# naver/panst3r

Measured on AMD Instinct MI355X. Metric: frames/sec (whole node), N-view 512px panoptic inference, higher is better.
Workload: dtype f16

## Files before the change

include/panst3r_hip.h:

```cpp
#ifndef PANST3R_HIP_H
#define PANST3R_HIP_H
#include <stdint.h>
#ifdef __cplusplus
extern "C" {
#endif

#define PST_ABI_VERSION 20

#define PST_BF16 0
#define PST_F32  1
#define PST_F16  2
#define PST_X3H  4

int pst_abi_version(void);
const char* pst_last_error(void);

typedef struct pst_gemm_params {
  const void* A;  int64_t lda;
  const void* W;  int64_t ldw;
  void* C;        int64_t ldc;
  int32_t M, N, K;
  const float* bias;
  const float* gamma;
  const float* res;  int64_t ldr;
  int32_t res_mod;
  int32_t act;
  int32_t out_fp32;
  int32_t trans_out;
  int32_t grp_in, grp_out, grp_off;
  int32_t ps_p, ps_c, ps_h, ps_w;
  int32_t conv_c, conv_h, conv_w;
  const void* zeros;
  const int32_t* rope_pos; const float* rope_cs; int32_t rope_hd;
  int32_t rope_npos;
  int32_t res_bf16;
  int32_t kernel;
  int32_t batch;
  int64_t a_bs, w_bs, c_bs, bias_bs;
  int32_t dtype16;
  void* xcopy; int64_t ldxc;
  float* stats_out; int32_t stats_ld;
  const float* ln_stats; int32_t ln_groups; const float* ln_colsum; float ln_eps;
  int32_t x3_block;
} pst_gemm_params;

int pst_gemm(const pst_gemm_params* p, void* stream);
const char* pst_gemm_variant(const pst_gemm_params* p);
int pst_gemm_pair(const pst_gemm_params* a, const pst_gemm_params* b, void* stream);
const char* pst_gemm_pair_variant(const pst_gemm_params* a, const pst_gemm_params* b);
#define PST_TUNE_G256_PP 3
#define PST_TUNE_PAIR 4
#define PST_TUNE_DEEP_RING 8
#define PST_TUNE_PAIR_ATTN 7
#define PST_TUNE_ATTN_XCD 9
#define PST_TUNE_CUS 10
#define PST_TUNE_PAIR_DELAY 6
#define PST_TUNE_DEPHASE 11
#define PST_TUNE_PAIR_RES 5
int pst_tune(int knob, int value);

int pst_mask_head_supported(int Q, int P, int C);
int pst_mask_head(const void* E, int64_t lde, const void* F, int64_t f_view_stride, float* out, int64_t out_view_stride, int nviews, int Q, int P, int C,
                  int dtype16, void* stream);

typedef struct pst_attn_params {
  const void* Q;  int64_t q_bs, q_hs, q_rs;
  const void* K;  int64_t k_bs, k_hs, k_rs;
  const void* Vt; int64_t v_bs, v_hs, v_ds;
  void* O;        int64_t o_bs, o_hs, o_rs;
  const uint8_t* mask; int64_t m_bs, m_rs;
// ... 154 lines not shown
```

panst3r_amd/csrc/gemm.hip:

```cpp
#include "common.h"
#include "../../include/panst3r_hip.h"

namespace pst {

int launch_gemm256(const pst_gemm_params& p, hipStream_t s);
int launch_gemm256p(const pst_gemm_params& p, hipStream_t s, int cus);
int gemm256p_pair_split(const pst_gemm_params& a, const pst_gemm_params& b, int cus, double separate_us, double* pair_us);
double gemm256p_single_us(const pst_gemm_params& p, int cus);
int launch_gemm256p_pair(const pst_gemm_params& a, const pst_gemm_params& b, hipStream_t s, int cus, int g0);
bool gemm256_persistent_ok(const pst_gemm_params& p);
int gemm256_persistent_class(const pst_gemm_params& p);
int gemm_f32_validate(const pst_gemm_params& p);
int launch_gemm_f32(const pst_gemm_params& p, hipStream_t s);
int rowstream_class(const pst_gemm_params& p);
int launch_rowstream(const pst_gemm_params& p, hipStream_t s, int cus);

constexpr int BK = 64;
constexpr int GROUP_M = 8;

template <int F>
__device__ __forceinline__ int perm_row(int row) {
  const int sub = row / (16 * F), rho = row - sub * (16 * F);
  const int f = rho >> 4, g = (rho >> 2) & 3, r = rho & 3;
  return sub * (16 * F) + g * (4 * F) + 4 * f + r;
// ... 38 lines not shown
    }
    uint4 rq[F32 ? 1 : NIT];
    if (!F32 && resb) {
#pragma unroll
      for (int it = 0; it < NIT; ++it) rq[F32 ? 0 : it] = *(const uint4*)((const bf16_t*)p.res + (int64_t)orow[it] * p.ldr + n);
    }
    if (rope) {
      constexpr int GRP = NIT < 4 ? NIT : 4;
#pragma unroll
      for (int g0 = 0; g0 < NIT; g0 += GRP) {
        float4 cs[GRP][4];
#pragma unroll
        for (int u = 0; u < GRP; ++u) rope_table(p, m0 + r0 + (g0 + u) * rstep, n, cs[u]);
#pragma unroll
        for (int u = 0; u < GRP; ++u) {
          const int r = r0 + (g0 + u) * rstep;
          const uint4 own = *(const uint4*)(smem + r * pitch + ((c ^ (r & (nch - 1))) << 4));
          const uint4 partner = *(const uint4*)(smem + r * pitch + (((c ^ 2) ^ (r & (nch - 1))) << 4));
          *(uint4*)((char*)p.C + ((int64_t)orow[g0 + u] * p.ldc + n) * 2) = rope_rotate<F16>(own, partner, cs[u], n);
        }
      }
      return;
    }
#pragma unroll
    for (int it = 0; it < NIT; ++it) {
      const int r = r0 + it * rstep;
      uint4 val = *(const uint4*)(smem + r * pitch + ((c ^ (r & (nch - 1))) << 4));
      if (F32 && pre) {
        float4 f = *(float4*)&val;
        const float4 q = resv[it];
        f.x += q.x; f.y += q.y; f.z += q.z; f.w += q.w;
        val = *(uint4*)&f;
      }
      float ssum = 0.f, ssq = 0.f;
      if (!F32 && resb) {
        uint32_t* w32 = (uint32_t*)&val;
        const uint32_t* q32 = (const uint32_t*)&rq[F32 ? 0 : it];
#pragma unroll
        for (int q = 0; q < 4; ++q) {
          w32[q] = H16<F16>::pack(H16<F16>::lo(w32[q]) + H16<F16>::lo(q32[q]), H16<F16>::hi(w32[q]) + H16<F16>::hi(q32[q]));
          if (p.stats_out) { ln_acc(H16<F16>::lo(w32[q]), ssum, ssq); ln_acc(H16<F16>::hi(w32[q]), ssum, ssq); }
        }
      } else if (!F32 && p.stats_out) {
        const uint32_t* w32 = (const uint32_t*)&val;
#pragma unroll
        for (int q = 0; q < 4; ++q) { ln_acc(H16<F16>::lo(w32[q]), ssum, ssq); ln_acc(H16<F16>::hi(w32[q]), ssum, ssq); }
      }
      if (F32) store_c4(p, orow[it], n, *(const float4*)&val);
      else *(uint4*)((char*)p.C + ((int64_t)orow[it] * p.ldc + n) * 2) = val;
      if (F32) {
        const float4 f = *(const float4*)&val;
        if (p.xcopy) *(uint2*)((bf16_t*)p.xcopy + (int64_t)orow[it] * p.ldxc + n) = make_uint2(H16<F16>::pack(f.x, f.y), H16<F16>::pack(f.z, f.w));
        if (p.stats_out) { float ss, sq; ln_acc4(f, ss, sq); ln_fold_stats<16>(p, ss, sq, c, orow[it], n); }
      } else if (p.stats_out) {
        ln_fold_stats<8>(p, ssum, ssq, c, orow[it], n);
      }
    }
    return;
  }
#pragma unroll
  for (int it = 0; it < (F32 ? BM / 8 : BM / 16); ++it) {
    const int r = tid / nch + it * rstep;
    const int m = m0 + r;
    if (r >= BM || m >= p.M || n >= p.N) continue;
    uint4 val = *(const uint4*)(smem + r * pitch + ((c ^ (r & (nch - 1))) << 4));
    if (p.rope_hd == 64 && !F32) val = rope_chunk<F16>(p, val, *(const uint4*)(smem + r * pitch + (((c ^ 2) ^ (r & (nch - 1))) << 4)), m, n);
    int orow = m;
    int64_t off;
    int ps_v = 0, ps_y = 0, ps_x = 0;
    if (p.ps_p > 0) {
      const int hw = p.ps_h * p.ps_w;
      ps_v = m / hw;
      const int tt = m - ps_v * hw;
      ps_y = tt / p.ps_w;
      ps_x = tt - ps_y * p.ps_w;
      const int dy = n / seg, rem = n - dy * seg;
      off = ((int64_t)(ps_v * p.ps_p * p.ps_h + p.ps_p * ps_y + dy) * p.ps_w + ps_x) * seg + rem;
    } else {
// ... 108 lines not shown
    if (p.conv_c > 0) {
      const int hw = p.conv_h * p.conv_w;
      const int img = m / hw, r = m - img * hw;
      const int y = r / p.conv_w;
      a_yx[j] = (y << 16) | (r - y * p.conv_w);
      a_src[j] = Ap + (int64_t)img * hw * p.conv_c;
    } else {
      a_yx[j] = 0;
      a_src[j] = Ap + (int64_t)m * p.lda;
    }
  }
#pragma unroll
  for (int j = 0; j < FN; ++j) {
    const int c = j * 256 + tid, lrow = c >> 3, pos = c & 7;
    b_sw[j] = ((pos ^ ((lrow >> 1) & 7)) << 3);
    const int row = TRANS ? lrow : perm_row<FN>(lrow);
    b_src[j] = Wp + (int64_t)min(n0 + row, p.N - 1) * p.ldw;
  }

  auto stage = [&](int kt, int buf) {
    const int k0 = kt * BK;
    char* a_dst = As + buf * (BM * 128) + wave * 1024;
    char* b_dst = Bs + buf * (BN * 128) + wave * 1024;
    if (p.conv_c > 0) {
      const int tap = k0 / p.conv_c, c0 = k0 - tap * p.conv_c;
      const int dy = tap / 3 - 1, dx = tap - (tap / 3) * 3 - 1;
#pragma unroll
      for (int j = 0; j < FM; ++j) {
        const int yy = (a_yx[j] >> 16) + dy, xx = (a_yx[j] & 0xffff) + dx;
        const bool ok = (yy >= 0) & (yy < p.conv_h) & (xx >= 0) & (xx < p.conv_w);
        const bf16_t* s = ok ? a_src[j] + ((int64_t)yy * p.conv_w + xx) * p.conv_c + c0 + a_sw[j]
                             : (const bf16_t*)p.zeros + a_sw[j];
        glds16(s, a_dst + j * 4096);
      }
    } else {
#pragma unroll
      for (int j = 0; j < FM; ++j) glds16(a_src[j] + k0 + a_sw[j], a_dst + j * 4096);
    }
#pragma unroll
    for (int j = 0; j < FN; ++j) glds16(b_src[j] + k0 + b_sw[j], b_dst + j * 4096);
  };

  f32x4 acc[FM][FN];
#pragma unroll
  for (int i = 0; i < FM; ++i)
#pragma unroll
    for (int j = 0; j < FN; ++j) acc[i][j] = f32x4{0.f, 0.f, 0.f, 0.f};
// ... 182 lines not shown
  hipLaunchKernelGGL((gemm_pair_kernel<FM, FN, NST, F16>), dim3(tma * tna + tmb * tnb), dim3(256), lds, s, a, tma * tna, tma, tna, b, tmb * tnb, tmb, tnb);
  return check_launch("gemm_pair");
}

template <int FM, int FN, bool TRANS, int NST, bool F16>
static int launch_t(const pst_gemm_params& p, hipStream_t s) {
  constexpr int BM = 32 * FM, BN = 32 * FN;
  const int tiles_m = (p.M + BM - 1) / BM, tiles_n = (p.N + BN - 1) / BN;
  const int tiles = tiles_m * tiles_n;
  const size_t lds = NST * (BM + BN) * 128 + BM * sizeof(float2);
  if constexpr (NST > 4) {
    static unsigned long long attr_seen = 0;
    once_per_device(attr_seen, [] { (void)hipFuncSetAttribute((const void*)gemm_kernel<FM, FN, TRANS, NST, F16>, hipFuncAttributeMaxDynamicSharedMemorySize, NST * (BM + BN) * 128 + BM * (int)sizeof(float2)); });
  }
  hipLaunchKernelGGL((gemm_kernel<FM, FN, TRANS, NST, F16>), dim3(tiles, p.batch > 1 ? p.batch : 1), dim3(256), lds, s, p, tiles, tiles_m, tiles_n);
  return check_launch("gemm");
}

template <int FM, int FN, bool TRANS, int NST>
static int launch(const pst_gemm_params& p, hipStream_t s) {
  return p.dtype16 == DT_F16 ? launch_t<FM, FN, TRANS, NST, true>(p, s) : launch_t<FM, FN, TRANS, NST, false>(p, s);
}

}

static int gemm_validate(const pst_gemm_params* pp) {
  using namespace pst;
  if (!pp) { set_error("gemm: null params"); return PST_EINVAL; }
  const pst_gemm_params& p = *pp;
  if (p.dtype16 == DT_F32) {
    if (p.M <= 0 || p.N <= 0 || p.K <= 0 || !p.A || !p.W || !p.C) { set_error("gemm: bad shape / null operand"); return PST_EINVAL; }
    if (p.kernel != 0) { set_error("gemm (fp32 operands): kernel must be 0"); return PST_EINVAL; }
    return pst::gemm_f32_validate(p);
  }
  if (p.dtype16 != DT_BF16 && p.dtype16 != DT_F16) { set_error("gemm: dtype16 must be PST_BF16, PST_F16 or PST_F32"); return PST_EINVAL; }
  if (p.act < 0 || p.act > 2) {
    set_error("gemm: act %d not available with 16-bit operands (0 none, 1 GELU(erf), 2 ReLU; 3 = GELU(tanh) needs fp32 operands)", p.act); return PST_EINVAL;
  }
  if (p.kernel != 0 && p.kernel != 128 && p.kernel != 256) { set_error("gemm: kernel must be 0 (auto), 128 or 256"); return PST_EINVAL; }
  if (p.kernel == 256 && (p.conv_c > 0 || (p.trans_out && pst::gemm256_persistent_class(p) != 3))) {
    set_error("gemm: the 256x256 kernel has no conv mode, and trans_out only in its persistent class (16-bit, ldc %% 8 == 0, N %% 64 == 0)"); return PST_EINVAL;
  }
  if (p.M <= 0 || p.N <= 0 || p.K <= 0) { set_error("gemm: bad shape M=%d N=%d K=%d", p.M, p.N, p.K); return PST_EINVAL; }
  if (p.K % 64 || p.N % 4) { set_error("gemm: need K%%64==0 and N%%4==0 (K=%d N=%d)", p.K, p.N); return PST_EINVAL; }
  if (!p.A || !p.W || !p.C) { set_error("gemm: null operand"); return PST_EINVAL; }
  if ((((uintptr_t)p.A | (uintptr_t)p.W) & 15) || ((uintptr_t)p.C & (p.out_fp32 ? 15 : 7))) {
    set_error("gemm: A/W must be 16-byte aligned, C 8-byte (bf16) / 16-byte (fp32) aligned"); return PST_EINVAL;
  }
  if ((p.ldw % 8) || (p.conv_c == 0 && (p.lda % 8))) { set_error("gemm: lda/ldw must be multiples of 8"); return PST_EINVAL; }
  if (p.conv_c > 0 && (p.conv_c % 64 || p.K != 9 * p.conv_c || !p.zeros || p.M % (p.conv_h * p.conv_w))) {
    set_error("gemm: bad conv mode (conv_c=%d K=%d)", p.conv_c, p.K); return PST_EINVAL;
  }
  if (p.ps_p > 0 && ((p.ps_p * p.ps_c) % 4 || p.N != p.ps_p * p.ps_p * p.ps_c || p.M % (p.ps_h * p.ps_w) || p.res || p.grp_in)) {
    set_error("gemm: bad pixel-shuffle store (p=%d c=%d N=%d)", p.ps_p, p.ps_c, p.N); return PST_EINVAL;
  }
  if (p.trans_out && (p.out_fp32 || p.res || p.gamma || p.grp_in || p.ps_p || (p.ldc % 4))) {
    set_error("gemm: trans_out supports bf16 + bias/act only, ldc%%4==0"); return PST_EINVAL;
  }
  if (!p.trans_out && !p.ps_p && (p.ldc % 4)) { set_error("gemm: ldc must be a multiple of 4"); return PST_EINVAL; }
  if (p.rope_hd != 0 && (p.rope_hd != 64 || p.out_fp32 || p.trans_out || p.ps_p || p.N % 64 || !p.rope_pos || !p.rope_cs || p.res)) {
    set_error("gemm: fused RoPE needs head dim 64, bf16 plain output, N%%64==0, no residual"); return PST_EINVAL;
  }
  if (p.res && (p.ldr % (p.res_bf16 ? 8 : 4))) { set_error("gemm: ldr must be a multiple of 4 (fp32) / 8 (bf16)"); return PST_EINVAL; }
  if (p.res && p.res_bf16 && ((uintptr_t)p.res & 15)) { set_error("gemm: bf16 residual must be 16-byte aligned"); return PST_EINVAL; }
  if ((p.stats_out || p.xcopy) && (p.N % 64 || p.ps_p || p.trans_out || p.res_mod || p.batch > 1 || (p.stats_out && p.stats_ld < p.N / 64) ||
                                   (p.xcopy && (!p.out_fp32 || p.ldxc % 4 || ((uintptr_t)p.xcopy & 7))))) {
    set_error("gemm: LayerNorm-fold producer outputs need a plain row-major store with N%%64==0 (xcopy: fp32 C only)"); return PST_EINVAL;
  }
  if (p.ln_stats && (!p.ln_colsum || p.ln_groups <= 0 || p.conv_c || p.batch > 1 || !(p.ln_eps > 0.f))) {
    set_error("gemm: LayerNorm-fold consumer needs ln_colsum, ln_groups > 0, ln_eps > 0 (no conv / batch mode)"); return PST_EINVAL;
  }
  if (p.x3_block && (!p.out_fp32 || p.dtype16 != DT_F16 || p.x3_block < p.N || p.x3_block % 4 || p.ldc < 3 * (int64_t)p.x3_block || p.ldc % 4 || p.ps_p || p.trans_out || p.xcopy ||
                     p.stats_out || p.batch > 1 || ((uintptr_t)p.C & 7))) {
    set_error("gemm: the split store (x3_block) needs out_fp32, f16 operands, x3_block >= N, ldc >= 3 x3_block, a plain row-major store"); return PST_EINVAL;
  }
  if (p.batch > 1 && (p.gamma || p.res || p.conv_c || p.rope_hd || p.ps_p || p.grp_in || p.kernel == 256 || p.batch > 65535 ||
                      (p.a_bs | p.w_bs | p.c_bs) % 8 || p.bias_bs % 4)) {
    set_error("gemm: strided batch supports bias/act/trans_out only, strides multiples of 8 elements (batch=%d)", p.batch); return PST_EINVAL;
  }
  return PST_OK;
}

static int g_deep_ring = 4;
namespace pst { int gemm256_pp(int set); int gemm256p_dephase(int set); int gemm256p_pair_delay(int set); int attn_pair_enable(int set); int attn_xcd_order(int set); }

static int gemm_choice(const pst_gemm_params& p) {
  const long big_tiles = (long)((p.M + 127) / 128) * ((p.N + 127) / 128) * (p.batch > 1 ? p.batch : 1);
  const bool small = p.kernel == 0 && big_tiles < (p.K >= 2048 ? 176 : 256);
  const long tiles256 = (long)((p.M + 255) / 256) * ((p.N + 255) / 256);
  const bool fits32 = (int64_t)p.M * p.lda < (1ll << 31) && (int64_t)p.N * p.ldw < (1ll << 31);
  const bool one_round = tiles256 >= 176 && tiles256 <= 256;
  if (p.trans_out) {
    const bool p3 = pst::gemm256_persistent_class(p) == 3 && fits32 && p.batch <= 1 && (p.kernel == 256 || (p.kernel == 0 && (tiles256 >= 384 || one_round) && p.K >= 512));
    return p3 ? 2 : (small ? 0 : 1);
  }
  const bool shape256 = p.N % 256 == 0 && p.K >= 1024 && (p.N >= 2048 || p.K >= 2048) && tiles256 >= 3 * 256 - 64;
  const int pclass = pst::gemm256_persistent_class(p);
  const bool shape256p = (tiles256 >= 384 || one_round) && ((pclass == 1 && p.K >= 512) || (pclass == 2 && (p.K >= 2048 || (p.K >= 768 && tiles256 <= 512))));
  if (p.conv_c == 0 && fits32 && p.batch <= 1 && (p.kernel == 256 || (p.kernel == 0 && (shape256 || shape256p)))) return 2;
  return small ? 0 : 1;
}

extern "C" int pst_gemm(const pst_gemm_params* pp, void* stream) {
  using namespace pst;
  if (int rc = gemm_validate(pp)) return rc;
  const pst_gemm_params& p = *pp;
  hipStream_t s = (hipStream_t)stream;
  if (p.dtype16 == DT_F32) return launch_gemm_f32(p, s);
  if (rowstream_class(p)) return launch_rowstream(p, s, num_cus());
  const int c = gemm_choice(p);
  if (c == 2) return gemm256_persistent_ok(p) ? launch_gemm256p(p, s, num_cus()) : launch_gemm256(p, s);
  if (p.trans_out) return c == 0 ? launch<2, 2, true, 4>(p, s) : launch<4, 4, true, 2>(p, s);
  if (c == 0 && g_deep_ring > 4 && p.batch <= 1) {
    const long tiles = (long)((p.M + 63) / 64) * ((p.N + 63) / 64);
    if (tiles <= num_cus() && p.K >= 512) return g_deep_ring >= 8 ? launch<2, 2, false, 8>(p, s) : launch<2, 2, false, 6>(p, s);
  }
  return c == 0 ? launch<2, 2, false, 4>(p, s) : launch<4, 4, false, 2>(p, s);
}

static bool pair_fusable(const pst_gemm_params& a, const pst_gemm_params& b) {
  using namespace pst;
  if (a.dtype16 == DT_F32 || a.dtype16 != b.dtype16 || a.trans_out || !b.trans_out || a.batch > 1 || b.batch > 1 || a.kernel || b.kernel) return false;
  if (rowstream_class(a) || rowstream_class(b)) return false;
  return gemm_choice(a) == 0 && gemm_choice(b) == 0;
}

static int g_pair_res = 1;
static int g_pair = 1;
static int pair_split_256p(const pst_gemm_params& a, const pst_gemm_params& b) {
  using namespace pst;
  if (!g_pair || a.dtype16 == DT_F32 || a.dtype16 != b.dtype16 || a.batch > 1 || b.batch > 1 || a.kernel || b.kernel) return 0;
  if (rowstream_class(a) || rowstream_class(b)) return 0;
  const int cus = num_cus();
  double sep = 0.0;
  const pst_gemm_params* ps[2] = {&a, &b};
  for (const pst_gemm_params* p : ps) {
    const bool fits32 = (int64_t)p->M * p->lda < (1ll << 31) && (int64_t)p->N * p->ldw < (1ll << 31);
    if (gemm_choice(*p) == 2 && gemm256_persistent_ok(*p)) { sep += gemm256p_single_us(*p, cus); continue; }
    const long tiles256 = (long)((p->M + 255) / 256) * ((p->N + 255) / 256);
    if (!(g_pair_res && gemm256_persistent_class(*p) == 2 && fits32 && p->conv_c == 0 && p->K >= 1024 && tiles256 >= 128)) return 0;
    sep += 2.0 * p->M * p->N * p->K / 470e6;
  }
  return gemm256p_pair_split(a, b, cus, sep, nullptr);
}

extern "C" int pst_gemm_pair(const pst_gemm_params* pa, const pst_gemm_params* pb, void* stream) {
  using namespace pst;
  if (int rc = gemm_validate(pa)) return rc;
  if (int rc = gemm_validate(pb)) return rc;
  hipStream_t s = (hipStream_t)stream;
  if (const int g0 = pair_split_256p(*pa, *pb)) return launch_gemm256p_pair(*pa, *pb, s, num_cus(), g0);
  if (!pair_fusable(*pa, *pb)) {
    if (int rc = pst_gemm(pa, stream)) return rc;
    return pst_gemm(pb, stream);
  }
  return pa->dtype16 == DT_F16 ? launch_pair_t<2, 2, 4, true>(*pa, *pb, s) : launch_pair_t<2, 2, 4, false>(*pa, *pb, s);
}

extern "C" const char* pst_gemm_pair_variant(const pst_gemm_params* pa, const pst_gemm_params* pb) {
  if (gemm_validate(pa) || gemm_validate(pb)) return nullptr;
  if (pair_split_256p(*pa, *pb)) return "gemm256p2_kernel";
  return pair_fusable(*pa, *pb) ? "gemm_pair_kernel<2,2>" : "";
}

extern "C" int pst_tune(int knob, int value) {
  if (knob == PST_TUNE_G256_PP) return pst::gemm256_pp(value);
  if (knob == PST_TUNE_PAIR_RES) { const int prev = g_pair_res; g_pair_res = value != 0; return prev; }
  if (knob == PST_TUNE_PAIR_DELAY) return pst::gemm256p_pair_delay(value);
  if (knob == PST_TUNE_DEPHASE) return pst::gemm256p_dephase(value);
  if (knob == PST_TUNE_PAIR_ATTN) return pst::attn_pair_enable(value);
  if (knob == PST_TUNE_ATTN_XCD) return pst::attn_xcd_order(value);
  if (knob == PST_TUNE_DEEP_RING) { const int prev = g_deep_ring; if (value == 4 || value == 6 || value == 8) g_deep_ring = value; return prev; }
  if (knob == PST_TUNE_PAIR) { const int prev = g_pair; g_pair = value != 0; return prev; }
  if (knob == PST_TUNE_CUS) { const int prev = pst::g_cu_budget; if (value >= 0 && value <= 1024) pst::g_cu_budget = value; return prev; }
  return -1;
}

extern "C" const char* pst_gemm_variant(const pst_gemm_params* pp) {
  if (gemm_validate(pp)) return nullptr;
  if (pp->dtype16 == pst::DT_F32) return "gemm_f32_kernel";
  if (pst::rowstream_class(*pp)) return "rowgemm384_kernel";
  const int c = gemm_choice(*pp);
  if (pp->trans_out && c != 2) return c == 0 ? "gemm_kernel<2,2,true>" : "gemm_kernel<4,4,true>";
  return c == 2 ? (pst::gemm256_persistent_ok(*pp) ? "gemm256p_kernel" : "gemm256_kernel") : (c == 0 ? "gemm_kernel<2,2,false>" : "gemm_kernel<4,4,false>");
}
```

panst3r_amd/hip.py:

```python
import ctypes as C
import os
import torch

_HERE = os.path.dirname(os.path.abspath(__file__))
LIB_PATH = os.environ.get('PST_LIB') or os.path.join(_HERE, 'lib', 'libpanst3r_hip.so')
ABI_VERSION = 20
STATS_BLOCKS = 128
_lib = None

i32, i64, f32, vp = C.c_int32, C.c_int64, C.c_float, C.c_void_p


class GemmParams(C.Structure):
    _fields_ = [('A', vp), ('lda', i64), ('W', vp), ('ldw', i64), ('C', vp), ('ldc', i64),
                ('M', i32), ('N', i32), ('K', i32),
                ('bias', vp), ('gamma', vp), ('res', vp), ('ldr', i64), ('res_mod', i32),
                ('act', i32), ('out_fp32', i32), ('trans_out', i32),
                ('grp_in', i32), ('grp_out', i32), ('grp_off', i32),
                ('ps_p', i32), ('ps_c', i32), ('ps_h', i32), ('ps_w', i32),
                ('conv_c', i32), ('conv_h', i32), ('conv_w', i32), ('zeros', vp), ('rope_pos', vp), ('rope_cs', vp), ('rope_hd', i32), ('rope_npos', i32), ('res_bf16', i32), ('kernel', i32),
                ('batch', i32), ('a_bs', i64), ('w_bs', i64), ('c_bs', i64), ('bias_bs', i64), ('dtype16', i32),
                ('xcopy', vp), ('ldxc', i64), ('stats_out', vp), ('stats_ld', i32), ('ln_stats', vp), ('ln_groups', i32), ('ln_colsum', vp), ('ln_eps', f32), ('x3_block', i32)]


class AttnParams(C.Structure):
    _fields_ = [('Q', vp), ('q_bs', i64), ('q_hs', i64), ('q_rs', i64),
                ('K', vp), ('k_bs', i64), ('k_hs', i64), ('k_rs', i64),
                ('Vt', vp), ('v_bs', i64), ('v_hs', i64), ('v_ds', i64),
                ('O', vp), ('o_bs', i64), ('o_hs', i64), ('o_rs', i64),
                ('mask', vp), ('m_bs', i64), ('m_rs', i64),
                ('B', i32), ('H', i32), ('Nq', i32), ('Nk', i32), ('hd', i32),
                ('scale', f32), ('zeros', vp), ('nsplit', i32), ('ws', vp), ('ws_bytes', i64), ('dtype16', i32), ('prescaled', i32)]


class CloudView(C.Structure):
    _fields_ = [('conf', vp), ('pts3d', vp), ('pts3d_local', vp), ('img', vp), ('pan', vp), ('offset', i64), ('npix', i32), ('first_wg', i32), ('c2w', f32 * 12)]


_CODES = {'i': C.c_int, 'l': C.c_int64, 'u': C.c_uint64, 'f': C.c_float, 'd': C.c_double, 'p': vp, 's': C.c_char_p,
          'G': C.POINTER(GemmParams), 'A': C.POINTER(AttnParams)}
SIGNATURES = {
    'pst_abi_version': 'i:', 'pst_last_error': 's:', 'pst_gemm': 'i:Gp', 'pst_gemm_variant': 's:G', 'pst_gemm_pair': 'i:GGp', 'pst_gemm_pair_variant': 's:GG',
    'pst_tune': 'i:ii', 'pst_mask_head_supported': 'i:iii', 'pst_mask_head': 'i:plplpliiiiip', 'pst_attn_workspace_bytes': 'l:iiiii', 'pst_attn_fwd': 'i:Ap',
    'pst_attn_variant': 's:A', 'pst_attn_pair': 'i:AAp', 'pst_attn_pair_variant': 's:AA', 'pst_layernorm': 'i:pliplippiifiiip',
    'pst_layernorm_add': 'i:pliplplippiifiiip', 'pst_token_embed': 'i:piipipiiplpp', 'pst_rowstats': 'i:pliplpiiiip',
    'pst_layernorm_add_batch': 'i:pliplplippiifiiiilllp', 'pst_split3': 'i:plpliiip', 'pst_split_operand': 'i:plpliiiiip', 'pst_split2': 'i:plppliiiip',
    'pst_transpose_f32': 'i:plpliip', 'pst_rope2d_split': 'i:plppppliiiip', 'pst_attn_x3': 'i:Apppilp', 'pst_attn_x3_variant': 's:A',
    'pst_rope2d': 'i:plppiiiip', 'pst_patchify': 'i:ppliiiiiip', 'pst_dino_preprocess': 'i:ppiiiiip', 'pst_image_prepare': 'i:piipiiiiiip',
    'pst_patch_rows': 'i:pplpliiiiiiip', 'pst_add_cast': 'i:plipliipliiip', 'pst_l2norm_rows': 'i:plpliifip', 'pst_mean4': 'i:ppiiiiip',
    'pst_resize_bilinear': 'i:ppiiiiiiip', 'pst_attn_mask_from_logits': 'i:plpliip', 'pst_loftup_guidance_gn': 'i:ppppfpppliiiiipp',
    'pst_loftup_minmax': 'i:ppiiip', 'pst_minmax_merge': 'i:pppip', 'pst_groupnorm_stats': 'i:plipiiiip', 'pst_groupnorm_apply': 'i:plippppliiiifiip',
    'pst_loftup_lr_pe': 'i:ppliiiiip', 'pst_pp_scores': 'i:piiffpppp', 'pst_pp_scores_softmax': 'i:piifpppp', 'pst_pp_sigmoid': 'i:pppiip',
    'pst_pp_argmax': 'i:pppiiiiifppppp', 'pst_pp_argmax_logits': 'i:pppiiiiifppppp', 'pst_pp_select': 'i:pppidppp', 'pst_pp_finalize': 'i:pppiffppp',
    'pst_qubo_upsample': 'i:ppiiiiip', 'pst_qubo_workspace_floats': 'l:il', 'pst_qubo_overlap': 'i:pilppp', 'pst_qubo_argmax': 'i:ppilppp',
    'pst_pointmap_activate': 'i:pppplip', 'pst_focal_weiszfeld': 'i:pppiiiip', 'pst_rigid_moments': 'i:ppppiifp', 'pst_retrieval_select': 'i:plppiiiplpp',
    'pst_retrieval_assign': 'i:plplpiiiiippppip', 'pst_retrieval_aggregate': 'i:plplpppiippp', 'pst_retrieval_scores': 'i:ppppppiiiiffpp',
    'pst_cloud_count': 'i:piifpp', 'pst_cloud_scan': 'i:pipp', 'pst_cloud_compact': 'i:piifppiffppppppp', 'pst_cloud_segment_median': 'i:ppplpiippppppp',
    'pst_qubo_anneal_max_n': 'i:', 'pst_qubo_anneal': 'i:piiifffuppppp',
    'pst_voxel_insert': 'i:plfplpppip', 'pst_voxel_count': 'i:pplpp', 'pst_voxel_rank': 'i:pplpppp', 'pst_voxel_accumulate': 'i:ppplfpppipppplppip',
    'pst_voxel_vote': 'i:pplpp', 'pst_voxel_emit': 'i:pppplfdppppiffppppppp',
    'pst_render_max_radius': 'i:', 'pst_render_splat': 'i:plpiiifiipip', 'pst_render_resolve': 'i:pllppppppppp',
}
EXPORTS = list(SIGNATURES)


# ... 179 lines not shown
    name = getattr(lib(), what)(*params)
    return name.decode() if name else unknown

_ZERO = {}


def zeros_page(device):
    z = _ZERO.get(device)
    if z is None:
        z = torch.zeros(256, dtype=torch.uint8, device=device)
        _ZERO[device] = z
    return z


def _rowmajor(t):
    assert t.dim() == 2 and t.stride(1) == 1, 'need a row-major 2-D view, got strides %s' % (t.stride(),)
    return t.stride(0)


ACT = {None: 0, 'none': 0, 'gelu': 1, 'relu': 2, 'gelu_tanh': 3}


def _gemm_params(a, w, out, bias=None, gamma=None, res=None, res_mod=0, act=None, trans_out=False, grp=None, ps=None, conv=None,
                 M=None, kernel=0, rope=None, batch=None, xcopy=None, stats_out=None, ln=None, x3_block=None):
    _dev(a, *FMT); _dev(w, *FMT); _dev(out, *FMT)
    p = GemmParams()
    p.dtype16 = _fmt(a, w) if a.dtype == torch.float32 else _same16(a, w, out, res)
    N, K = w.shape
    if conv is not None:
        cc, ch, cw = conv
        p.conv_c, p.conv_h, p.conv_w = cc, ch, cw
        Mv = a.numel() // cc
        p.lda = cc
        assert K == 9 * cc
    else:
        Mv = a.shape[0] if M is None else M
        assert a.shape[1] == K, (a.shape, w.shape)
        p.lda = _rowmajor(a)
    p.A, p.W, p.C = _ptr(a), _ptr(w), _ptr(out)
    p.ldw = _rowmajor(w)
    p.M, p.N, p.K = Mv, N, K
    p.zeros = _ptr(zeros_page(a.device))
    if ps is not None:
        p.ps_p, p.ps_c, p.ps_h, p.ps_w = ps
        p.ldc = 0
    else:
        p.ldc = _rowmajor(out)
    if bias is not None:
        p.bias = _ptr(_dev(bias, torch.float32))
    if gamma is not None:
        p.gamma = _ptr(_dev(gamma, torch.float32))
    if res is not None:
        p.res, p.ldr, p.res_mod = _ptr(_dev(res, torch.float32, *H16)), _rowmajor(res), res_mod
        p.res_bf16 = int(res.dtype in H16)
    if batch is not None:
        p.batch, p.a_bs, p.w_bs, p.c_bs, p.bias_bs = batch
    p.act = ACT[act]
    p.out_fp32 = int(out.dtype == torch.float32)
    if x3_block:
        assert out.dtype == X3_FMT and out.shape[1] >= 3 * x3_block
        p.out_fp32, p.x3_block = 1, int(x3_block)
    p.trans_out = int(trans_out)
    p.kernel = kernel
    if rope is not None:
        p.rope_pos, p.rope_cs, p.rope_hd = _ptr(_dev(rope[0], torch.int32)), _ptr(_dev(rope[1], torch.float32)), 64
        p.rope_npos = int(rope[1].shape[0])
    if grp is not None:
        p.grp_in, p.grp_out, p.grp_off = grp
    if xcopy is not None:
        p.xcopy, p.ldxc = _ptr(_dev(xcopy, a.dtype)), _rowmajor(xcopy)
    if stats_out is not None:
        assert stats_out.dtype == torch.float32 and stats_out.dim() == 3 and stats_out.shape[2] == 2 and stats_out.is_contiguous()
        p.stats_out, p.stats_ld = _ptr(_dev(stats_out)), stats_out.shape[1]
    if ln is not None:
        st, cs, eps = ln
        assert st.dtype == torch.float32 and st.dim() == 3 and st.shape[2] == 2 and st.is_contiguous() and st.shape[1] * 64 >= K
        p.ln_stats, p.ln_groups, p.ln_colsum, p.ln_eps = _ptr(_dev(st)), K // 64, _ptr(_dev(cs, torch.float32)), float(eps)
        assert K % 64 == 0 and st.shape[1] == K // 64, 'LayerNorm fold: the statistics must cover exactly the K columns of A'
    tag = (Mv, N, K, 'f32' if out.dtype == torch.float32 else '16', act or '', 'res' if res is not None else '',
           'grp' if grp is not None else '', 'rope' if rope is not None else '', 'conv' if conv is not None else '', 'ps' if ps is not None else '')
    return p, 2.0 * Mv * N * K * (batch[0] if batch else 1), tag


X3 = True
X3_FMT = torch.float16
X3H = 4


def split_operand(x, side, kpad=None, out=None, fmt=None):
    _dev(x, torch.float32)
    rows, K = x.shape
    kpad = (K + 63) // 64 * 64 if kpad is None else kpad
    if out is None:
        out = torch.empty(rows, 3 * kpad, dtype=fmt or X3_FMT, device=x.device)
    _call('pst_split_operand', _ptr(x), _rowmajor(x), _ptr(out), _rowmajor(out), rows, K, kpad, side, _tc(out))
    return out


def split2(x, transpose=False, hi=None, lo=None, fmt=None):
    _dev(x, torch.float32)
    rows, K = x.shape
# ... 70 lines not shown
        kw['conv'] = (3 * c64(cc), ch, cw)
    else:
        kpad = w.shape[1] // 3
        if w.shape[1] != 3 * kpad or kpad % 64 or a.shape[1] > kpad:
            raise RuntimeError('fp32-operand GEMM: a 16-bit W next to an fp32 A must be a split-packed weight [N, 3 Kpad] with Kpad >= K (A %s, W %s)'
                               % (tuple(a.shape), tuple(w.shape)))
        rows = a.shape[0] if kw.get('M') is None else kw['M']
        src = a[:rows]
        if batch is not None:
            count, a_bs, w_bs, c_bs, bias_bs = batch
            lda = _rowmajor(a)
            if a_bs != rows * lda:
                raise RuntimeError('fp32-operand GEMM: batched A problems must be stacked row blocks')
            src = a.as_strided((count * rows, a.shape[1]), (lda, 1))
            kw['batch'] = batch = (count, rows * 3 * kpad, w_bs, c_bs, bias_bs)
            kw['M'] = rows
        a3 = split_operand(src, 0, kpad=kpad, fmt=fmt)
    finish = None
    if kw.get('trans_out'):
        out, kw, finish = _trans_f32(a3.shape[0] // (batch[0] if batch else 1), w.shape[0], out, kw)
    return a3, w, out, kw, finish


def gemm(a, w, out, **kw):
    if _x3_wanted(a, w):
        a3, w3, o3, kw3, finish = _x3_prepare(a, w, out, kw)
        gemm(a3, w3, o3, **kw3)
        if finish is not None:
            finish()
        return out
    if kw.get('trans_out') and out.dtype == torch.float32 and a.dtype in H16:
        o3, kw3, finish = _trans_f32(a.shape[0] if kw.get('M') is None else kw['M'], w.shape[0], out, kw)
        gemm(a, w, o3, **kw3)
        finish()
        return out
    p, flops, tag = _gemm_params(a, w, out, **kw)
    _timed(lambda: _variant('pst_gemm_variant', 'gemm?', p), flops, tag, _call, 'pst_gemm', p)
    if MAXABS is not None and TIMER is None:
        _note_gemm(out, kw, tag)
    return out


def _note_gemm(out, kw, tag):
    M, N = int(tag[0]), int(tag[1])
    what = 'gemm N=%d K=%s%s' % (N, tag[2], (' ' + kw['act']) if kw.get('act') else '')
    if kw.get('ps') or kw.get('grp') or kw.get('batch') or kw.get('conv'):
# ... 717 lines not shown
```

panst3r_amd/model/panoptic.py:

```python
import math
import os
import torch
import torch.nn as nn

from .. import hip
from .common import (HipModule, qscale, Packed, Layout, adt, empty, attn_out, mlp_hidden, x3, vit_block, pack_croco_block, pack_norm, f32, ParamLinear,
                     grid_pos, ceil_to, grow_table, Stream, fold_ln, ln_of)
from .params import BlockP, MlpP, CrossAttnP, MHAP

VIEW_CHUNK = 16
BALANCED_CHUNKS = os.environ.get('PST_BALANCED_CHUNKS', '1') != '0'


def view_chunks(V):
    n = (V + VIEW_CHUNK - 1) // VIEW_CHUNK
    v0 = 0
    for i in range(n):
        c = (V // n + (1 if i < V % n else 0)) if BALANCED_CHUNKS else min(VIEW_CHUNK, V - v0)
        yield v0, c
        v0 += c


class InputMixer(HipModule):
    def __init__(self, img_size, patch_size, in_dim, hidden_dim, num_heads=12, num_layers=3, ff_dim_mult=4):
# ... 113 lines not shown
    def __init__(self, input_dim, dim, output_stride=2, patch_size=16, color_feats=True, n_freqs=20, num_heads=4, num_layers=2,
                 lr_pe_type='sine'):
        super().__init__()
        assert lr_pe_type == 'sine' and color_feats and output_stride == 2, 'released LoftUp configuration only'
        self.input_dim, self.dim, self.patch_size, self.n_freqs, self.num_heads = input_dim, dim, patch_size, n_freqs, num_heads
        self.patch_embed = nn.Conv2d(input_dim, input_dim, kernel_size=1)
        start = 5 * n_freqs * 2 + 3
        self.start_dim = start
        self.lr_pe = _Featurizer(2, 5)
        self.lr_input_proj = nn.Sequential(ParamLinear(input_dim + 20, dim), nn.LayerNorm(dim))
        self.fourier_feat = nn.Sequential(nn.Identity(), _Featurizer(5, n_freqs))
        self.first_conv = nn.Sequential(nn.GroupNorm(1, start), nn.Conv2d(start, dim, 3, padding=1), nn.GroupNorm(8, dim), nn.ReLU(),
                                        nn.Conv2d(dim, dim, 3, padding=1), nn.GroupNorm(8, dim), nn.ReLU())
        self.ca_transformer_blocks = nn.ModuleList([_CrossOnlyP(dim, 1) for _ in range(num_layers)])
        self.ca_transformer_norm = nn.LayerNorm(dim)
        self.mask_dim, self.fpn_dim = dim, input_dim

    def _pack(self, device):
        def conv_w(conv, cpad):
            wt = conv.weight.detach().float().permute(0, 2, 3, 1)
            out = torch.zeros(wt.shape[0], 3, 3, cpad)
            out[..., :wt.shape[-1]] = wt
            return Packed(out.reshape(wt.shape[0], -1), conv.bias, device, taps=9)
        c0 = ceil_to(self.start_dim, 64)
        fc = self.first_conv
        blocks = []
        for b in self.ca_transformer_blocks:
            c = b.cross_attn
            blocks.append(dict(norm2=pack_norm(b.norm2, device), norm3=pack_norm(b.norm3, device), norm_y=pack_norm(b.norm_y, device),
                               q=fold_ln(c.projq.weight, c.projq.bias, b.norm2, device), k=Packed(c.projk.weight, c.projk.bias, device),
                               v=Packed(c.projv.weight, c.projv.bias, device), proj=Packed(c.proj.weight, c.proj.bias, device),
                               fc1=fold_ln(b.mlp.fc1.weight, b.mlp.fc1.bias, b.norm3, device), fc2=Packed(b.mlp.fc2.weight, b.mlp.fc2.bias, device)))
        gn = lambda g: (f32(g.weight, device), f32(g.bias, device), float(g.eps))
        return dict(pe=Packed(self.patch_embed.weight, self.patch_embed.bias, device), c0=c0,
                    lr_bias=f32(self.lr_pe.biases, device), ff_bias=f32(self.fourier_feat[1].biases, device),
                    lr_proj=Packed(self.lr_input_proj[0].weight, self.lr_input_proj[0].bias, device),
                    lr_norm=pack_norm(self.lr_input_proj[1], device),
                    gn0=gn(fc[0]), conv1=conv_w(fc[1], c0), gn1=gn(fc[2]), conv2=conv_w(fc[4], self.dim), gn2=gn(fc[5]),
                    blocks=blocks, norm=pack_norm(self.ca_transformer_norm, device))

    def lr_width(self):
        return ceil_to(self.input_dim + 20, 64)

    @torch.no_grad()
    def guidance_tokens(self, imgs, h, w, mm=None):
        dev = imgs.device
        pk = self.packed(dev)
        C = self.dim
        if h > w:
            imgs = imgs.transpose(2, 3).contiguous()
        V = imgs.shape[0]
        H2, W2 = imgs.shape[2] // 2, imgs.shape[3] // 2
        P = H2 * W2
        out = empty(V * P, C, adt(), dev)
        for v0, n in view_chunks(V):
            st0 = hip.stats_buffer(n, 1, dev)
            g0 = empty(n * P, pk['c0'], adt(), dev)
            scratch = torch.empty(n * (3 * P + 6) + 16, dtype=torch.float32, device=dev)
            hip.loftup_guidance_gn(imgs[v0:v0 + n].contiguous(), pk['ff_bias'], pk['gn0'][0], pk['gn0'][1], pk['gn0'][2], scratch, st0, g0,
                                   self.n_freqs, mm=None if mm is None else mm[v0:v0 + n].contiguous())
            del scratch
            c1 = empty(n * P, C, adt(), dev)
            hip.gemm(g0, pk['conv1'].w, c1, bias=pk['conv1'].b, conv=(pk['c0'], H2, W2))
            st = hip.stats_buffer(n, 8, dev)
            hip.groupnorm_stats(c1, st, n, P, C, 8)
            g1 = out[v0 * P:(v0 + n) * P]
            if x3():
                g1s = torch.empty(n * P, 3 * C, dtype=hip.X3_FMT, device=dev)
                hip.groupnorm_apply(c1, st, pk['gn1'][0], pk['gn1'][1], g1s, n, P, C, 8, pk['gn1'][2], True, split=True)
                hip.gemm(g1s, pk['conv2'].w, c1, bias=pk['conv2'].b, conv=(3 * C, H2, W2))
                del g1s
            else:
                hip.groupnorm_apply(c1, st, pk['gn1'][0], pk['gn1'][1], g1, n, P, C, 8, pk['gn1'][2], True)
                hip.gemm(g1, pk['conv2'].w, c1, bias=pk['conv2'].b, conv=(C, H2, W2))
            hip.groupnorm_stats(c1, st, n, P, C, 8)
            hip.groupnorm_apply(c1, st, pk['gn2'][0], pk['gn2'][1], g1, n, P, C, 8, pk['gn2'][2], True)
            del g0, c1
        return out

    @torch.no_grad()
    def upscale_tokens(self, lr, imgs, V, h, w, fpn_out, mask_out, guidance=None, mm=None):
        dev = lr.device
        pk = self.packed(dev)
        T, D, C, Hh = h * w, self.input_dim, self.dim, self.num_heads
        hd = C // Hh
        H2, W2 = (imgs.shape[3] // 2, imgs.shape[2] // 2) if h > w else (imgs.shape[2] // 2, imgs.shape[3] // 2)
        assert tuple(mask_out.shape) == (V, H2, W2, C), (tuple(mask_out.shape), (V, H2, W2, C))
        P = H2 * W2
        if guidance is None:
            guidance = self.guidance_tokens(imgs, h, w, mm=mm)
        assert tuple(guidance.shape) == (V * P, C)
        hip.gemm(lr[:, :D], pk['pe'].w, fpn_out, bias=pk['pe'].b)
        lr[:, D:].zero_()
        hip.loftup_lr_pe(pk['lr_bias'], lr, D, V, h, w)
        lay = Layout(V, T)
        kv = torch.zeros(lay.rows, C, dtype=torch.float32, device=dev)
        hip.gemm(lr, pk['lr_proj'].w, kv, bias=pk['lr_proj'].b, grp=lay.grp)
        kvn = empty(lay.rows, C, torch.float32, dev)
# ... 610 lines not shown
```

Before: 331.3.

## Fuse GroupNorm statistics into conv GEMM epilogue and shrink first-conv channel padding

The implicit-conv GEMM epilogue now accumulates per-tile, per-group sum and sum-of-squares into a partial buffer, and a small fold kernel reduces those partials into per-view GroupNorm statistics. This removes separate groupnorm_stats passes over the LoFTUp guidance conv outputs. The conv loader also gains a path for channel counts that are multiples of 8 rather than 64, so the first conv pads start_dim to 8 instead of 64 and does less K work. In exchange the epilogue does extra shared-memory reduction work, and each fused conv adds an extra small fold launch and scratch allocations.

```diff
diff --git a/include/panst3r_hip.h b/include/panst3r_hip.h
--- a/include/panst3r_hip.h
+++ b/include/panst3r_hip.h
@@ -42,10 +42,12 @@
   float* stats_out; int32_t stats_ld;
   const float* ln_stats; int32_t ln_groups; const float* ln_colsum; float ln_eps;
   int32_t x3_block;
+  float* gn_stats; float* gn_part; int32_t gn_groups, gn_p;
 } pst_gemm_params;
 
 int pst_gemm(const pst_gemm_params* p, void* stream);
 const char* pst_gemm_variant(const pst_gemm_params* p);
+int64_t pst_gemm_gn_floats(const pst_gemm_params* p);
 int pst_gemm_pair(const pst_gemm_params* a, const pst_gemm_params* b, void* stream);
 const char* pst_gemm_pair_variant(const pst_gemm_params* a, const pst_gemm_params* b);
 #define PST_TUNE_G256_PP 3
diff --git a/panst3r_amd/csrc/gemm.hip b/panst3r_amd/csrc/gemm.hip
--- a/panst3r_amd/csrc/gemm.hip
+++ b/panst3r_amd/csrc/gemm.hip
@@ -84,6 +84,15 @@
       }
       return;
     }
+    constexpr int GN_RPS = 32 / rstep, GN_SLOTS = NIT / 2, GN_NSC = BN / 64;
+    float4 gns[F32 ? 1 : GN_SLOTS];
+    int gn_next[BM / 64];
+    if (!F32 && p.gn_part) {
+#pragma unroll
+      for (int q = 0; q < GN_SLOTS; ++q) gns[F32 ? 0 : q] = make_float4(0.f, 0.f, 0.f, 0.f);
+#pragma unroll
+      for (int sb = 0; sb < BM / 64; ++sb) gn_next[sb] = ((m0 + 64 * sb) / p.gn_p + 1) * p.gn_p;
+    }
 #pragma unroll
     for (int it = 0; it < NIT; ++it) {
       const int r = r0 + it * rstep;
@@ -108,6 +117,17 @@
 #pragma unroll
         for (int q = 0; q < 4; ++q) { ln_acc(H16<F16>::lo(w32[q]), ssum, ssq); ln_acc(H16<F16>::hi(w32[q]), ssum, ssq); }
       }
+      if constexpr (!F32) if (p.gn_part) {
+        const uint32_t* w32 = (const uint32_t*)&val;
+        float s8 = 0.f, q8 = 0.f;
+#pragma unroll
+        for (int q = 0; q < 4; ++q) { ln_acc(H16<F16>::lo(w32[q]), s8, q8); ln_acc(H16<F16>::hi(w32[q]), s8, q8); }
+        const int sb = it / (2 * GN_RPS), slot = sb * GN_RPS + (it % (2 * GN_RPS)) % GN_RPS;
+        const bool second = m0 + r >= gn_next[sb];
+        float4& a = gns[F32 ? 0 : slot];
+        a.x += second ? 0.f : s8; a.y += second ? 0.f : q8;
+        a.z += second ? s8 : 0.f; a.w += second ? q8 : 0.f;
+      }
       if (F32) store_c4(p, orow[it], n, *(const float4*)&val);
       else *(uint4*)((char*)p.C + ((int64_t)orow[it] * p.ldc + n) * 2) = val;
       if (F32) {
@@ -116,6 +136,31 @@
         if (p.stats_out) { float ss, sq; ln_acc4(f, ss, sq); ln_fold_stats<16>(p, ss, sq, c, orow[it], n); }
       } else if (p.stats_out) {
         ln_fold_stats<8>(p, ssum, ssq, c, orow[it], n);
+      }
+    }
+    if constexpr (!F32) if (p.gn_part) {
+      float4* gsc = (float4*)(smem + BM * pitch);
+#pragma unroll
+      for (int q = 0; q < GN_SLOTS; ++q) {
+        const int sb = q / GN_RPS, rs = r0 + rstep * (q % GN_RPS);
+        gsc[((sb * GN_NSC + (c >> 3)) * 32 + rs) * 8 + (c & 7)] = gns[F32 ? 0 : q];
+      }
+      __syncthreads();
+      const int G = p.gn_groups;
+      if (tid < (BM / 64) * GN_NSC * 4 * G) {
+        const int st = tid / (4 * G), rem = tid - st * 4 * G;
+        const int sb = st / GN_NSC, sc = st - sb * GN_NSC;
+        const int half = rem / (2 * G), grp = (rem >> 1) % G, comp = rem & 1;
+        const int cpg = (p.N / G) >> 3;
+        const int cb = (n0 >> 3) + 8 * sc;
+        const int c_lo = max(grp * cpg - cb, 0), c_hi = min((grp + 1) * cpg - cb, 8);
+        const float* gf = (const float*)(gsc + st * 256) + 2 * half + comp;
+        float a = 0.f;
+        for (int cc = c_lo; cc < c_hi; ++cc)
+#pragma unroll 4
+          for (int rs = 0; rs < 32; ++rs) a += gf[4 * (rs * 8 + cc)];
+        const int64_t tile = (int64_t)(m0 / 64 + sb) * (p.N / 64) + (n0 >> 6) + sc;
+        p.gn_part[((tile * 2 + half) * G + grp) * 2 + comp] = a;
       }
     }
     return;
@@ -270,7 +315,18 @@
     const int k0 = kt * BK;
     char* a_dst = As + buf * (BM * 128) + wave * 1024;
     char* b_dst = Bs + buf * (BN * 128) + wave * 1024;
-    if (p.conv_c > 0) {
+    if (p.conv_c > 0 && (p.conv_c & 63)) {
+      const int k = k0 + a_sw[0];
+      const int tap = k / p.conv_c, c0 = k - tap * p.conv_c;
+      const int dy = tap / 3 - 1, dx = tap - (tap / 3) * 3 - 1;
+#pragma unroll
+      for (int j = 0; j < FM; ++j) {
+        const int yy = (a_yx[j] >> 16) + dy, xx = (a_yx[j] & 0xffff) + dx;
+        const bool ok = (tap < 9) & (yy >= 0) & (yy < p.conv_h) & (xx >= 0) & (xx < p.conv_w);
+        const bf16_t* s = ok ? a_src[j] + ((int64_t)yy * p.conv_w + xx) * p.conv_c + c0 : (const bf16_t*)p.zeros + a_sw[j];
+        glds16(s, a_dst + j * 4096);
+      }
+    } else if (p.conv_c > 0) {
       const int tap = k0 / p.conv_c, c0 = k0 - tap * p.conv_c;
       const int dy = tap / 3 - 1, dx = tap - (tap / 3) * 3 - 1;
 #pragma unroll
@@ -499,6 +555,42 @@
   return p.dtype16 == DT_F16 ? launch_t<FM, FN, TRANS, NST, true>(p, s) : launch_t<FM, FN, TRANS, NST, false>(p, s);
 }
 
+__global__ __launch_bounds__(256) void gn_fold_kernel(const float* part, float* stats, int P, int BM, int tiles_n, int G) {
+  __shared__ float sh[256];
+  const int view = blockIdx.x, slots = 2 * G, nparts = 256 / slots;
+  const int slot = threadIdx.x % slots, pn = threadIdx.x / slots;
+  const int tm_lo = (int)(((int64_t)view * P) / BM), tm_hi = (int)((((int64_t)view + 1) * P - 1) / BM);
+  const int n = (tm_hi - tm_lo + 1) * tiles_n;
+  float a = 0.f;
+  if (pn < nparts) {
+    for (int e = pn; e < n; e += nparts) {
+      const int tr = e / tiles_n, tm = tm_lo + tr, tn = e - tr * tiles_n;
+      const int half = (int)(((int64_t)tm * BM) / P) == view ? 0 : 1;
+      a += part[(((int64_t)tm * tiles_n + tn) * 2 + half) * slots + slot];
+    }
+  }
+  sh[threadIdx.x] = a;
+  __syncthreads();
+  if ((int)threadIdx.x < slots) {
+    float t = 0.f;
+    for (int q = 0; q < nparts; ++q) t += sh[q * slots + threadIdx.x];
+    stats[(int64_t)view * slots + threadIdx.x] = t;
+  }
+}
+
+}
+
+static int gemm_choice(const pst_gemm_params& p);
+
+static int gn_tile(const pst_gemm_params& p) {
+  using namespace pst;
+  if (p.dtype16 == DT_F32 || p.out_fp32 || p.trans_out || p.ps_p || p.grp_in || p.res || p.res_mod || p.rope_hd || p.stats_out || p.xcopy || p.ln_stats ||
+      p.batch > 1 || p.x3_block) return 0;
+  if (p.gn_groups <= 0 || p.gn_groups > 16 || p.gn_p < 64 || p.M % p.gn_p || p.N % (8 * p.gn_groups) || (p.ldc & 7) || ((uintptr_t)p.C & 15)) return 0;
+  if (p.M % 64 || p.N % 64 || rowstream_class(p)) return 0;
+  const int c = gemm_choice(p);
+  if (c == 2) return 0;
+  return (c == 1 && p.M % 128 == 0 && p.N % 128 == 0) ? 128 : 64;
 }
 
 static int gemm_validate(const pst_gemm_params* pp) {
@@ -525,8 +617,8 @@
     set_error("gemm: A/W must be 16-byte aligned, C 8-byte (bf16) / 16-byte (fp32) aligned"); return PST_EINVAL;
   }
   if ((p.ldw % 8) || (p.conv_c == 0 && (p.lda % 8))) { set_error("gemm: lda/ldw must be multiples of 8"); return PST_EINVAL; }
-  if (p.conv_c > 0 && (p.conv_c % 64 || p.K != 9 * p.conv_c || !p.zeros || p.M % (p.conv_h * p.conv_w))) {
-    set_error("gemm: bad conv mode (conv_c=%d K=%d)", p.conv_c, p.K); return PST_EINVAL;
+  if (p.conv_c > 0 && (p.conv_c % 8 || p.K != (9 * p.conv_c + 63) / 64 * 64 || !p.zeros || p.M % (p.conv_h * p.conv_w) || p.conv_h > 32767 || p.conv_w > 32767)) {
+    set_error("gemm: bad conv mode (conv_c=%d K=%d: conv_c %% 8 == 0, K = 9 conv_c rounded up to 64)", p.conv_c, p.K); return PST_EINVAL;
   }
   if (p.ps_p > 0 && ((p.ps_p * p.ps_c) % 4 || p.N != p.ps_p * p.ps_p * p.ps_c || p.M % (p.ps_h * p.ps_w) || p.res || p.grp_in)) {
     set_error("gemm: bad pixel-shuffle store (p=%d c=%d N=%d)", p.ps_p, p.ps_c, p.N); return PST_EINVAL;
@@ -550,6 +642,10 @@
   if (p.x3_block && (!p.out_fp32 || p.dtype16 != DT_F16 || p.x3_block < p.N || p.x3_block % 4 || p.ldc < 3 * (int64_t)p.x3_block || p.ldc % 4 || p.ps_p || p.trans_out || p.xcopy ||
                      p.stats_out || p.batch > 1 || ((uintptr_t)p.C & 7))) {
     set_error("gemm: the split store (x3_block) needs out_fp32, f16 operands, x3_block >= N, ldc >= 3 x3_block, a plain row-major store"); return PST_EINVAL;
+  }
+  if (p.gn_stats && (!p.gn_part || !gn_tile(p))) {
+    set_error("gemm: GroupNorm statistics need a 16-bit plain row-major C with M %% 64 == 0, N %% 64 == 0, gn_p >= 64, M %% gn_p == 0, gn_groups <= 16, "
+              "N %% (8 gn_groups) == 0 (M=%d N=%d gn_p=%d gn_groups=%d); ask pst_gemm_gn_floats first", p.M, p.N, p.gn_p, p.gn_groups); return PST_EINVAL;
   }
   if (p.batch > 1 && (p.gamma || p.res || p.conv_c || p.rope_hd || p.ps_p || p.grp_in || p.kernel == 256 || p.batch > 65535 ||
                       (p.a_bs | p.w_bs | p.c_bs) % 8 || p.bias_bs % 4)) {
@@ -588,6 +684,11 @@
   const int c = gemm_choice(p);
   if (c == 2) return gemm256_persistent_ok(p) ? launch_gemm256p(p, s, num_cus()) : launch_gemm256(p, s);
   if (p.trans_out) return c == 0 ? launch<2, 2, true, 4>(p, s) : launch<4, 4, true, 2>(p, s);
+  if (p.gn_stats) {
+    if (int rc = gn_tile(p) == 64 ? launch<2, 2, false, 4>(p, s) : launch<4, 4, false, 2>(p, s)) return rc;
+    hipLaunchKernelGGL(gn_fold_kernel, dim3(p.M / p.gn_p), dim3(256), 0, s, p.gn_part, p.gn_stats, p.gn_p, 64, p.N / 64, p.gn_groups);
+    return check_launch("gn_fold");
+  }
   if (c == 0 && g_deep_ring > 4 && p.batch <= 1) {
     const long tiles = (long)((p.M + 63) / 64) * ((p.N + 63) / 64);
     if (tiles <= num_cus() && p.K >= 512) return g_deep_ring >= 8 ? launch<2, 2, false, 8>(p, s) : launch<2, 2, false, 6>(p, s);
@@ -625,6 +726,7 @@
   using namespace pst;
   if (int rc = gemm_validate(pa)) return rc;
   if (int rc = gemm_validate(pb)) return rc;
+  if (pa->gn_stats || pb->gn_stats) { set_error("gemm_pair: no GroupNorm statistics in a shared launch"); return PST_EINVAL; }
   hipStream_t s = (hipStream_t)stream;
   if (const int g0 = pair_split_256p(*pa, *pb)) return launch_gemm256p_pair(*pa, *pb, s, num_cus(), g0);
   if (!pair_fusable(*pa, *pb)) {
@@ -653,11 +755,20 @@
   return -1;
 }
 
+extern "C" int64_t pst_gemm_gn_floats(const pst_gemm_params* pp) {
+  if (!pp) return 0;
+  pst_gemm_params p = *pp;
+  p.gn_stats = nullptr; p.gn_part = nullptr;
+  if (gemm_validate(&p)) return 0;
+  return gn_tile(p) ? (int64_t)(p.M / 64) * (p.N / 64) * 4 * p.gn_groups : 0;
+}
+
 extern "C" const char* pst_gemm_variant(const pst_gemm_params* pp) {
   if (gemm_validate(pp)) return nullptr;
   if (pp->dtype16 == pst::DT_F32) return "gemm_f32_kernel";
   if (pst::rowstream_class(*pp)) return "rowgemm384_kernel";
   const int c = gemm_choice(*pp);
+  if (pp->gn_stats) return gn_tile(*pp) == 64 ? "gemm_kernel<2,2,false>" : "gemm_kernel<4,4,false>";
   if (pp->trans_out && c != 2) return c == 0 ? "gemm_kernel<2,2,true>" : "gemm_kernel<4,4,true>";
   return c == 2 ? (pst::gemm256_persistent_ok(*pp) ? "gemm256p_kernel" : "gemm256_kernel") : (c == 0 ? "gemm_kernel<2,2,false>" : "gemm_kernel<4,4,false>");
 }
diff --git a/panst3r_amd/hip.py b/panst3r_amd/hip.py
--- a/panst3r_amd/hip.py
+++ b/panst3r_amd/hip.py
@@ -20,7 +20,8 @@
                 ('ps_p', i32), ('ps_c', i32), ('ps_h', i32), ('ps_w', i32),
                 ('conv_c', i32), ('conv_h', i32), ('conv_w', i32), ('zeros', vp), ('rope_pos', vp), ('rope_cs', vp), ('rope_hd', i32), ('rope_npos', i32), ('res_bf16', i32), ('kernel', i32),
                 ('batch', i32), ('a_bs', i64), ('w_bs', i64), ('c_bs', i64), ('bias_bs', i64), ('dtype16', i32),
-                ('xcopy', vp), ('ldxc', i64), ('stats_out', vp), ('stats_ld', i32), ('ln_stats', vp), ('ln_groups', i32), ('ln_colsum', vp), ('ln_eps', f32), ('x3_block', i32)]
+                ('xcopy', vp), ('ldxc', i64), ('stats_out', vp), ('stats_ld', i32), ('ln_stats', vp), ('ln_groups', i32), ('ln_colsum', vp), ('ln_eps', f32), ('x3_block', i32),
+                ('gn_stats', vp), ('gn_part', vp), ('gn_groups', i32), ('gn_p', i32)]
 
 
 class AttnParams(C.Structure):
@@ -40,7 +41,7 @@
 _CODES = {'i': C.c_int, 'l': C.c_int64, 'u': C.c_uint64, 'f': C.c_float, 'd': C.c_double, 'p': vp, 's': C.c_char_p,
           'G': C.POINTER(GemmParams), 'A': C.POINTER(AttnParams)}
 SIGNATURES = {
-    'pst_abi_version': 'i:', 'pst_last_error': 's:', 'pst_gemm': 'i:Gp', 'pst_gemm_variant': 's:G', 'pst_gemm_pair': 'i:GGp', 'pst_gemm_pair_variant': 's:GG',
+    'pst_abi_version': 'i:', 'pst_last_error': 's:', 'pst_gemm': 'i:Gp', 'pst_gemm_variant': 's:G', 'pst_gemm_gn_floats': 'l:G', 'pst_gemm_pair': 'i:GGp', 'pst_gemm_pair_variant': 's:GG',
     'pst_tune': 'i:ii', 'pst_mask_head_supported': 'i:iii', 'pst_mask_head': 'i:plplpliiiiip', 'pst_attn_workspace_bytes': 'l:iiiii', 'pst_attn_fwd': 'i:Ap',
     'pst_attn_variant': 's:A', 'pst_attn_pair': 'i:AAp', 'pst_attn_pair_variant': 's:AA', 'pst_layernorm': 'i:pliplippiifiiip',
     'pst_layernorm_add': 'i:pliplplippiifiiip', 'pst_token_embed': 'i:piipipiiplpp', 'pst_rowstats': 'i:pliplpiiiip',
@@ -266,7 +267,7 @@
 
 
 def _gemm_params(a, w, out, bias=None, gamma=None, res=None, res_mod=0, act=None, trans_out=False, grp=None, ps=None, conv=None,
-                 M=None, kernel=0, rope=None, batch=None, xcopy=None, stats_out=None, ln=None, x3_block=None):
+                 M=None, kernel=0, rope=None, batch=None, xcopy=None, stats_out=None, ln=None, x3_block=None, gn=None):
     _dev(a, *FMT); _dev(w, *FMT); _dev(out, *FMT)
     p = GemmParams()
     p.dtype16 = _fmt(a, w) if a.dtype == torch.float32 else _same16(a, w, out, res)
@@ -276,7 +277,7 @@
         p.conv_c, p.conv_h, p.conv_w = cc, ch, cw
         Mv = a.numel() // cc
         p.lda = cc
-        assert K == 9 * cc
+        assert K == (9 * cc + 63) // 64 * 64, (K, cc)
     else:
         Mv = a.shape[0] if M is None else M
         assert a.shape[1] == K, (a.shape, w.shape)
@@ -321,6 +322,14 @@
         assert st.dtype == torch.float32 and st.dim() == 3 and st.shape[2] == 2 and st.is_contiguous() and st.shape[1] * 64 >= K
         p.ln_stats, p.ln_groups, p.ln_colsum, p.ln_eps = _ptr(_dev(st)), K // 64, _ptr(_dev(cs, torch.float32)), float(eps)
         assert K % 64 == 0 and st.shape[1] == K // 64, 'LayerNorm fold: the statistics must cover exactly the K columns of A'
+    if gn is not None:
+        st, part, G, P = gn
+        _dev(st, torch.float32); _dev(part, torch.float32)
+        assert st.is_contiguous() and part.is_contiguous() and st.numel() >= Mv // P * G * 2
+        p.gn_groups, p.gn_p = G, P
+        need = int(lib().pst_gemm_gn_floats(C.byref(p)))
+        assert 0 < need <= part.numel(), 'GroupNorm statistics from the epilogue: unsupported shape or short scratch (%d floats needed)' % need
+        p.gn_stats, p.gn_part = _ptr(st), _ptr(part)
     tag = (Mv, N, K, 'f32' if out.dtype == torch.float32 else '16', act or '', 'res' if res is not None else '',
            'grp' if grp is not None else '', 'rope' if rope is not None else '', 'conv' if conv is not None else '', 'ps' if ps is not None else '')
     return p, 2.0 * Mv * N * K * (batch[0] if batch else 1), tag
@@ -437,6 +446,13 @@
     return a3, w, out, kw, finish
 
 
+def gemm_gn_scratch(a, w, out, G, P, **kw):
+    p, _, _ = _gemm_params(a, w, out, **kw)
+    p.gn_groups, p.gn_p = G, P
+    n = int(lib().pst_gemm_gn_floats(C.byref(p)))
+    return torch.empty(n, dtype=torch.float32, device=out.device) if n > 0 else None
+
+
 def gemm(a, w, out, **kw):
     if _x3_wanted(a, w):
         a3, w3, o3, kw3, finish = _x3_prepare(a, w, out, kw)
diff --git a/panst3r_amd/model/panoptic.py b/panst3r_amd/model/panoptic.py
--- a/panst3r_amd/model/panoptic.py
+++ b/panst3r_amd/model/panoptic.py
@@ -159,7 +159,7 @@
             out = torch.zeros(wt.shape[0], 3, 3, cpad)
             out[..., :wt.shape[-1]] = wt
             return Packed(out.reshape(wt.shape[0], -1), conv.bias, device, taps=9)
-        c0 = ceil_to(self.start_dim, 64)
+        c0 = ceil_to(self.start_dim, 8 if adt() in (torch.float16, torch.bfloat16) else 64)
         fc = self.first_conv
         blocks = []
         for b in self.ca_transformer_blocks:
@@ -198,19 +198,28 @@
                                    self.n_freqs, mm=None if mm is None else mm[v0:v0 + n].contiguous())
             del scratch
             c1 = empty(n * P, C, adt(), dev)
-            hip.gemm(g0, pk['conv1'].w, c1, bias=pk['conv1'].b, conv=(pk['c0'], H2, W2))
             st = hip.stats_buffer(n, 8, dev)
-            hip.groupnorm_stats(c1, st, n, P, C, 8)
+            part = None if x3() else hip.gemm_gn_scratch(g0, pk['conv1'].w, c1, 8, P, bias=pk['conv1'].b, conv=(pk['c0'], H2, W2))
+            if part is not None:
+                hip.gemm(g0, pk['conv1'].w, c1, bias=pk['conv1'].b, conv=(pk['c0'], H2, W2), gn=(st, part, 8, P))
+            else:
+                hip.gemm(g0, pk['conv1'].w, c1, bias=pk['conv1'].b, conv=(pk['c0'], H2, W2))
+                hip.groupnorm_stats(c1, st, n, P, C, 8)
             g1 = out[v0 * P:(v0 + n) * P]
             if x3():
                 g1s = torch.empty(n * P, 3 * C, dtype=hip.X3_FMT, device=dev)
                 hip.groupnorm_apply(c1, st, pk['gn1'][0], pk['gn1'][1], g1s, n, P, C, 8, pk['gn1'][2], True, split=True)
                 hip.gemm(g1s, pk['conv2'].w, c1, bias=pk['conv2'].b, conv=(3 * C, H2, W2))
                 del g1s
+                hip.groupnorm_stats(c1, st, n, P, C, 8)
             else:
                 hip.groupnorm_apply(c1, st, pk['gn1'][0], pk['gn1'][1], g1, n, P, C, 8, pk['gn1'][2], True)
-                hip.gemm(g1, pk['conv2'].w, c1, bias=pk['conv2'].b, conv=(C, H2, W2))
-            hip.groupnorm_stats(c1, st, n, P, C, 8)
+                part2 = hip.gemm_gn_scratch(g1, pk['conv2'].w, c1, 8, P, bias=pk['conv2'].b, conv=(C, H2, W2))
+                if part2 is not None:
+                    hip.gemm(g1, pk['conv2'].w, c1, bias=pk['conv2'].b, conv=(C, H2, W2), gn=(st, part2, 8, P))
+                else:
+                    hip.gemm(g1, pk['conv2'].w, c1, bias=pk['conv2'].b, conv=(C, H2, W2))
+                    hip.groupnorm_stats(c1, st, n, P, C, 8)
             hip.groupnorm_apply(c1, st, pk['gn2'][0], pk['gn2'][1], g1, n, P, C, 8, pk['gn2'][2], True)
             del g0, c1
         return out
```

Result: no change. 328.4 (-0.9%).
